# NinV/Background-Debiased-Video-CIL

Measured on AMD Instinct MI355X. Metric: clips/sec fwd+bwd TSM-R50 8x224^2 bs32/GPU, higher is better.
Workload: dtype f32; 1 GPU; TSM-ResNet50 fwd+bwd+SGD step, synthetic 32x8x3x224x224 clips per GPU, 101 classes, SimpleLinear+CrossEntropyLoss, dropout 0.5, random-init weights; fp32 tensors, accumulators and results; conv products: fp32 via 3xbf16 split, 6 MFMA products, fp32 accumulate (dropped terms <= 2^-24 relative); conv_arith=bf16x3, clips_per_gpu=32, global_batch=32, parallelism=dp1

## Files before the change

### background-debiased-video-cil_amd/_lib.py

```python
from __future__ import annotations

import ctypes
import os
from ctypes import POINTER, Structure, c_char_p, c_float, c_int, c_int32, c_int64, c_size_t, c_uint16, c_uint64, c_void_p

_HERE = os.path.dirname(os.path.abspath(__file__))
_OVERRIDE = os.environ.get('BDVCIL_LIB_PATH')
LIB_PATH = _OVERRIDE or os.path.join(_HERE, 'csrc', 'libbdvcil_hip.so')
ABI_VERSION = 32

_lib = None


class ConvGeom(Structure):
    _fields_ = [(n, c_int32) for n in
                ('N', 'H', 'W', 'Cin', 'Ho', 'Wo', 'Cout', 'R', 'S', 'stride', 'pad', 'T', 'fold', 'pad_w', 'Rt', 'st_t', 'act_dtype')]

    def key(self):
        return tuple(getattr(self, n) for n, _ in self._fields_)


P = c_void_p
_F3 = c_float * 3

# ... 2 lines not shown
    _fields_ = [('scale', c_void_p), ('shift', c_void_p), ('residual', c_void_p), ('relu', c_int32)]


class BnStatFuse(Structure):
    _fields_ = [('y', c_void_p), ('relu_mask', c_void_p), ('mean', c_void_p), ('invstd', c_void_p), ('partial', c_void_p),
                ('relu_scale', c_void_p), ('relu_shift', c_void_p)]

class JpegInfo(Structure):
    _fields_ = [('width', c_int32), ('height', c_int32), ('ncomp', c_int32), ('h', c_int32 * 3), ('v', c_int32 * 3),
                ('blocks_w', c_int32 * 3), ('blocks_h', c_int32 * 3), ('down_w', c_int32 * 3), ('down_h', c_int32 * 3),
                ('qt', (c_uint16 * 64) * 3), ('coef_offset', c_int64 * 3), ('coef_count', c_int64)]

    def geometry_key(self):
        return (self.width, self.height, self.ncomp, tuple(self.h), tuple(self.v))


SIGNATURES = {
    'bdv_last_error': (c_char_p, []),
    'bdv_abi_version': (c_int, []),
    'bdv_source_hash': (c_char_p, []),
    'bdv_conv_workspace_bytes': (c_size_t, [POINTER(ConvGeom), c_int]),
    'bdv_conv_fprop_stat_rows': (c_int, [POINTER(ConvGeom)]),
    'bdv_conv_fprop': (c_int, [P, P, P, POINTER(ConvGeom), P, POINTER(ConvAffine), P, c_size_t, P]),
    'bdv_conv_fprop_x3': (c_int, [P, P, P, POINTER(ConvGeom), P, POINTER(ConvAffine), P, c_size_t, P]),
    'bdv_conv_dgrad_stat_rows': (c_int, [POINTER(ConvGeom)]),
    'bdv_conv_dgrad': (c_int, [P, P, P, P, P, POINTER(ConvGeom), POINTER(BnStatFuse), P, c_size_t, P]),
    'bdv_conv_dgrad_x3': (c_int, [P, P, P, P, P, P, POINTER(ConvGeom), POINTER(BnStatFuse), P, c_size_t, P]),
    'bdv_conv_weight_planes_bytes': (c_size_t, [POINTER(ConvGeom)]),
    'bdv_conv_split_weights': (c_int, [P, POINTER(ConvGeom), P, P, P]),
    'bdv_conv_fprop_pre_ok': (c_int, [POINTER(ConvGeom)]),
    'bdv_conv_fprop_pre_stat_rows': (c_int, [POINTER(ConvGeom)]),
    'bdv_conv_wgrad_pre_ok': (c_int, [POINTER(ConvGeom)]),
    'bdv_conv_debug_force_tile': (c_int, [c_int]),
    'bdv_conv_uses_planes': (c_int, [POINTER(ConvGeom), c_int, c_int]),
    'bdv_conv_kernel_name': (c_int, [POINTER(ConvGeom), c_int, c_int, c_char_p, c_size_t]),
    'bdv_conv_fprop_pl_stat_rows': (c_int, [POINTER(ConvGeom), c_int]),
    'bdv_conv_dgrad_pl_stat_rows': (c_int, [POINTER(ConvGeom), c_int]),
    'bdv_conv_fprop_pl': (c_int, [P, P, P, P, POINTER(ConvGeom), P, POINTER(ConvAffine), P, c_size_t, c_int, P, P, P]),
    'bdv_conv_dgrad_pl': (c_int, [P, P, P, P, P, P, POINTER(ConvGeom), POINTER(BnStatFuse), P, c_size_t, c_int, P]),
    'bdv_conv_wgrad': (c_int, [P, P, P, c_float, POINTER(ConvGeom), P, c_size_t, P]),
    'bdv_conv_wgrad_splits': (c_int, [POINTER(ConvGeom)]),
    'bdv_conv_wgrad_partial': (c_int, [P, P, POINTER(ConvGeom), P, c_size_t, P]),
    'bdv_conv_wgrad_partial_x3': (c_int, [P, P, POINTER(ConvGeom), P, c_size_t, P]),
    'bdv_conv_wgrad_pl_splits': (c_int, [POINTER(ConvGeom)]),
    'bdv_conv_wgrad_partial_pl': (c_int, [P, P, POINTER(ConvGeom), P, c_size_t, c_int, P, P, P]),
    'bdv_wgrad_reduce_batched': (c_int, [P, P, P, P, c_int, c_float, P]),
    'bdv_bn_workspace_bytes': (c_size_t, [c_int64, c_int]),
    'bdv_bn_train_stats': (c_int, [P, c_int64, c_int, P, P, c_float, c_float, P, P, P, P, P, P, P, c_size_t, P]),
    'bdv_bn_train_finalize': (c_int, [P, c_int, c_int64, c_int, P, P, c_float, c_float, P, P, P, P, P, P, P]),
    'bdv_bn_eval_params': (c_int, [c_int, P, P, P, P, c_float, P, P, P]),
    'bdv_bn_apply': (c_int, [P, P, P, P, P, P, P, P, c_int64, c_int, c_int, c_int, P]),
    'bdv_bn_backward': (c_int, [P, P, P, P, P, P, P, P, P, c_float, c_int64, c_int, c_int, P, c_int, P, P, P, c_size_t, c_int, P]),
    'bdv_bn_finalize_scratch_bytes': (c_size_t, [c_int]),
    'bdv_bn_finalize_splits': (c_int, [c_int, c_int]),
    'bdv_bn_train_finalize_split': (c_int, [P, c_int, c_int64, c_int, P, P, c_float, c_float, P, P, P, P, P, P, c_int, P, c_size_t, P]),
    'bdv_bn_backward_split': (c_int, [P, P, P, P, P, P, P, P, P, c_float, c_int64, c_int, c_int, P, c_int, P, P, P, c_size_t, c_int,
                                      c_int, P, c_size_t, P]),
    'bdv_bn_pair_workspace_bytes': (c_size_t, [c_int64, c_int]),
    'bdv_bn_backward_pair': (c_int, [P, P, P, P, P, P, P, c_int, P, P, P, P, P, P, P, P, P, P, c_int64, c_int, P, c_size_t, c_int, c_int,
                                     P, c_size_t, P]),
    'bdv_bn_eval_backward': (c_int, [P, P, P, P, P, P, P, P, P, P, P, c_float, c_int64, c_int, P, c_size_t, c_int, c_int, P, c_size_t, P]),
    'bdv_bn_backward_maxpool_split': (c_int, [P, P, P, P, P, P, P, P, P, P, c_float, c_int, c_int, c_int, c_int, P, c_size_t, c_int,
                                              c_int, P, c_size_t, P]),
    'bdv_bn_backward_maxpool': (c_int, [P, P, P, P, P, P, P, P, P, P, c_float, c_int, c_int, c_int, c_int, P, c_size_t, c_int, P]),
    'bdv_relu_bwd': (c_int, [P, P, P, P, c_int64, c_int, P]),
    'bdv_add': (c_int, [P, P, P, c_int64, c_int, P]),
# ... 28 lines not shown
    'bdv_lsc_bwd': (c_int, [P, P, P, P, P, P, P, P, c_float, P, c_int, c_int, c_int, c_int, P]),
    'bdv_linear_fwd': (c_int, [P, P, P, P, c_int, c_int, c_int, P]),
    'bdv_linear_bwd': (c_int, [P, P, P, P, P, P, c_float, c_int, c_int, c_int, P]),
    'bdv_consensus_fwd': (c_int, [P, P, c_int, c_int, c_int, P]),
    'bdv_consensus_bwd': (c_int, [P, P, c_int, c_int, c_int, P]),
    'bdv_dropout': (c_int, [P, P, c_int64, c_float, c_uint64, P]),
    'bdv_lsc_loss': (c_int, [P, P, P, c_float, c_int, P, P, P, P, c_int, c_int, P]),
    'bdv_softce_loss': (c_int, [P, P, P, P, P, c_int, c_int, P]),
    'bdv_icarl_targets': (c_int, [P, P, c_int, P, P, c_int, c_int, P]),
    'bdv_acm_targets': (c_int, [P, P, P, c_float, P, c_int, c_int, P]),
    'bdv_softmax_mean': (c_int, [P, P, c_int, c_int, c_int, c_int, P]),
    'bdv_topk_acc': (c_int, [P, P, P, c_int, c_int, P]),
    'bdv_repr_from_features': (c_int, [P, P, P, c_int, c_int, c_int, c_int, P]),
    'bdv_nme_workspace_bytes': (c_size_t, [c_int, c_int]),
    'bdv_nme_classify': (c_int, [P, P, P, P, c_int, c_int, c_int, c_int, P, c_size_t, P]),
    'bdv_class_means': (c_int, [P, P, P, c_int, c_int, c_int, P]),
    'bdv_herding_workspace_bytes': (c_size_t, [c_int, c_int]),
    'bdv_herding_select': (c_int, [P, c_int, c_int, c_int, c_int, P, P, P, P, c_size_t, P]),
    'bdv_randaug_workspace_bytes': (c_size_t, [c_int, c_int, c_int, c_int]),
    'bdv_randaug_apply': (c_int, [P, P, P, P, c_int, c_int, c_int, c_int, P, c_size_t, P]),
    'bdv_reduce_workspace_bytes': (c_size_t, []),
    'bdv_kd_mse_fwd': (c_int, [P, P, P, c_int64, P, c_size_t, c_int, P]),
    'bdv_kd_mse_bwd': (c_int, [P, P, P, c_float, P, c_int64, c_int, P]),
    'bdv_multi_sqnorm': (c_int, [P, P, c_int, P, P, c_size_t, P]),
    'bdv_clip_coef': (c_int, [P, c_float, c_float, P, P]),
    'bdv_multi_sgd': (c_int, [P, P, P, P, P, P, c_int, c_float, c_float, P, P]),
}


class HipExtensionError(RuntimeError):
    pass


HASHED_SOURCES = ('conv_mfma.hip', 'bn.hip', 'pool_frontend.hip', 'head_loss.hip', 'repr.hip', 'augment.hip', 'optim.hip', 'jpeg.hip',
                  'background.hip', 'actor_cut_mix.hip', 'sim_cam.hip', 'api_common.cpp', 'common.h', 'resize_linear.h', 'Makefile', '../../include/bdvcil_hip.h')


def source_hash():
    import hashlib
    h = hashlib.sha256()
    base = os.path.join(_HERE, 'csrc')
    for name in HASHED_SOURCES:
        path = os.path.join(base, name)
        if not os.path.exists(path):
            return None
        with open(path, 'rb') as f:
            h.update(f.read())
    return h.hexdigest()


def lib():
    global _lib
    if _lib is None:
        if not os.path.exists(LIB_PATH):
            raise HipExtensionError(
                f'HIP extension not built: {LIB_PATH} is missing. Run `python -c "import __graft_entry__ as g; '
                f'g.build()"` (or `make -C {os.path.dirname(LIB_PATH)}`). There is no CPU fallback.')
        handle = ctypes.CDLL(LIB_PATH)
        for name, (res, args) in SIGNATURES.items():
            fn = getattr(handle, name)
            fn.restype = res
            fn.argtypes = args
        if handle.bdv_abi_version() != ABI_VERSION:
            raise HipExtensionError(f'ABI mismatch: library {handle.bdv_abi_version()} != binding {ABI_VERSION}')
        want, have = source_hash(), handle.bdv_source_hash().decode()
        if want is not None and want != have and not _OVERRIDE:
            raise HipExtensionError(f'stale library: {LIB_PATH} was built from other sources (hash {have[:12]}, in-tree '
                                    f'{want[:12]}). Rebuild: make -C {os.path.dirname(LIB_PATH)}')
# ... 9 lines not shown
```

### background-debiased-video-cil_amd/csrc/conv_mfma.hip

```cpp
#include <stdlib.h>
#include "common.h"

#ifdef BDV_STAMPS
__device__ unsigned long long* g_stamp_buf = nullptr;
__device__ int g_stamp_cap = 0;
#define BDV_STAMP(slot)                                                                                                          \
  do {                                                                                                                           \
    if (threadIdx.x == 0 && g_stamp_buf != nullptr && (int)(blockIdx.x + gridDim.x * blockIdx.y) < g_stamp_cap) {                 \
      unsigned long long* q_ = g_stamp_buf + (size_t)(blockIdx.x + gridDim.x * blockIdx.y) * 8;                                  \
      if ((slot) == 4) asm volatile("s_waitcnt vmcnt(0)" ::: "memory");                                                          \
      q_[slot] = __builtin_amdgcn_s_memtime();                                                                                   \
      if ((slot) == 0) { q_[5] = __builtin_amdgcn_s_memrealtime(); q_[7] = __builtin_amdgcn_s_getreg((4 << 0) | (0 << 6) | (31 << 11)); } \
      if ((slot) == 4) q_[6] = __builtin_amdgcn_s_memrealtime();                                                                 \
    }                                                                                                                            \
  } while (0)
#else
#define BDV_STAMP(slot) do { } while (0)
#endif

namespace {

constexpr int BK = 32;

struct Geom {
  int N, H, W, Cin, Ho, Wo, Cout, R, S, stride, pad, pad_w, T, fold;
  int Rt, st_t;
  float rcp_RS, rcp_S;
  int M;
  int Ktot;
  float rcp_HoWo, rcp_Wo;
  int stagger;
};

typedef unsigned int u32x4 __attribute__((ext_vector_type(4)));
// ... 558 lines not shown
      ra[p] = buf_load16(xr, (a_base[p] + koff_a + cls * frame_bytes) | (v ? 0 : kOOB), 0);
    }
#pragma unroll
    for (int p = 0; p < BP; ++p) rb[p] = buf_load16(wr, b_base[p], koff_b);
    s += 1;
    const int ws_ = (s == g.S) ? 1 : 0;
    s = ws_ ? 0 : s;
    r += ws_;
    const int wr_ = (r == g.R) ? 1 : 0;
    r = wr_ ? 0 : r;
    chunk += wr_;
  };

  f32x16 acc[TM][TN];
  zero_acc<TM, TN>(acc);

  load();
  for (int kt = it.kb; kt < it.ke; ++kt) {
    __syncthreads();
    store_transposed<LDA, AP>(As, ra, tid);
    store_transposed<LDB, BP>(Bs, rb, tid);
    __syncthreads();
    if (kt + 1 < it.ke) load();
    mma_stage<LDA, LDB, TM, TN, 32 * WM, 32 * WN, true, true>(As, Bs, acc, wm0, wn0, lane);
  }

  if (it.pslot >= 0) {
    store_partial<TM, TN>(slab, it.pslot, acc, tid);
    return;
  }
  fprop_epilogue<BM, BN, WM, WN>(acc, smem, y, g, epi, mt, nt, tid);
}

typedef __bf16 bf16x8_t __attribute__((ext_vector_type(8)));
typedef __bf16 bf16x4_t __attribute__((ext_vector_type(4)));
typedef float f32x4_t __attribute__((ext_vector_type(4)));
constexpr int X3_LDK = BK + 8;

typedef __bf16 bf16x2_t __attribute__((ext_vector_type(2)));
typedef float f32x2_t __attribute__((ext_vector_type(2)));
typedef unsigned u32x2_t __attribute__((ext_vector_type(2)));
__device__ __forceinline__ unsigned pack_bf16x2(float a, float b) {
  return __builtin_bit_cast(unsigned, __builtin_convertvector((f32x2_t){a, b}, bf16x2_t));
}
__device__ __forceinline__ u32x2_t bf16_hi_pairs(const float4 v) { return (u32x2_t){pack_bf16x2(v.x, v.y), pack_bf16x2(v.z, v.w)}; }
__device__ __forceinline__ void split3_pairs(const float4 v, u32x2_t& hi, u32x2_t& mid, u32x2_t& lo) {
  const unsigned h0 = pack_bf16x2(v.x, v.y), h1 = pack_bf16x2(v.z, v.w);
  const float rx = v.x - __uint_as_float(h0 << 16), ry = v.y - __uint_as_float(h0 & 0xffff0000u);
  const float rz = v.z - __uint_as_float(h1 << 16), rw = v.w - __uint_as_float(h1 & 0xffff0000u);
  const unsigned m0 = pack_bf16x2(rx, ry), m1 = pack_bf16x2(rz, rw);
  const float sx = rx - __uint_as_float(m0 << 16), sy = ry - __uint_as_float(m0 & 0xffff0000u);
  const float sz = rz - __uint_as_float(m1 << 16), sw = rw - __uint_as_float(m1 & 0xffff0000u);
  hi = (u32x2_t){h0, h1};
  mid = (u32x2_t){m0, m1};
  lo = (u32x2_t){pack_bf16x2(sx, sy), pack_bf16x2(sz, sw)};
}

template <int ROWS, int P>
__device__ __forceinline__ void store_split3(unsigned short* __restrict__ dst, const float4 (&v)[P], int tid) {
  const int arow = tid >> 3, kg = tid & 7;
#pragma unroll
  for (int p = 0; p < P; ++p) {
    u32x2_t hi, mid, lo;
    split3_pairs(v[p], hi, mid, lo);
    unsigned short* q = dst + (arow + 32 * p) * X3_LDK + 4 * kg;
    *reinterpret_cast<u32x2_t*>(q) = hi;
    *reinterpret_cast<u32x2_t*>(q + ROWS * X3_LDK) = mid;
    *reinterpret_cast<u32x2_t*>(q + 2 * ROWS * X3_LDK) = lo;
  }
}

template <int TM, int TN, int MS, int NS, int ROWS_A, int ROWS_B>
__device__ __forceinline__ void mma_stage_x3(const unsigned short* __restrict__ As, const unsigned short* __restrict__ Bs,
                                             f32x16 (&acc)[TM][TN], int wm0, int wn0, int lane) {
  const int r = lane & 31, h = lane >> 5;
#pragma unroll
  for (int s = 0; s < BK / 16; ++s) {
    bf16x8_t a[3][TM], b[3][TN];
#pragma unroll
    for (int p = 0; p < 3; ++p) {
#pragma unroll
      for (int i = 0; i < TM; ++i)
        a[p][i] = *reinterpret_cast<const bf16x8_t*>(As + (p * ROWS_A + wm0 + MS * i + r) * X3_LDK + 16 * s + 8 * h);
#pragma unroll
      for (int j = 0; j < TN; ++j)
        b[p][j] = *reinterpret_cast<const bf16x8_t*>(Bs + (p * ROWS_B + wn0 + NS * j + r) * X3_LDK + 16 * s + 8 * h);
    }
#pragma unroll
    for (int i = 0; i < TM; ++i)
// ... 998 lines not shown
    float4* d = reinterpret_cast<float4*>(dw) + i;
    if (beta != 0.f) {
      const float4 o = *d;
      s.x += beta * o.x;
      s.y += beta * o.y;
      s.z += beta * o.z;
      s.w += beta * o.w;
    }
    *d = s;
  }
}

__global__ __launch_bounds__(256) void wgrad_reduce_kernel(const float* __restrict__ slab, float* __restrict__ dw, float beta,
                                                            int splits, int64_t numel4) {
  wgrad_reduce_block(slab, dw, beta, splits, numel4, blockIdx.x);
}

struct ReduceBatch {
  const float* slab[BDV_MAX_REDUCE_ITEMS];
  float* dw[BDV_MAX_REDUCE_ITEMS];
  int splits[BDV_MAX_REDUCE_ITEMS];
  int numel4[BDV_MAX_REDUCE_ITEMS];
  int first_block[BDV_MAX_REDUCE_ITEMS + 1];
  int n;
};

__global__ __launch_bounds__(256) void wgrad_reduce_batched_kernel(ReduceBatch rb, float beta) {
  int k = 0;
  while (k + 1 < rb.n && (int)blockIdx.x >= rb.first_block[k + 1]) ++k;
  wgrad_reduce_block(rb.slab[k], rb.dw[k], beta, rb.splits[k], rb.numel4[k], blockIdx.x - rb.first_block[k]);
}


__device__ __forceinline__ int pl_off(int row, int c) { return row * 64 + ((c ^ ((row >> 2) & 3)) << 4); }

__device__ __forceinline__ void pl_split_store(unsigned char* __restrict__ base, int plane_bytes, int row, int kg, const float4 v) {
  u32x2_t hi, mid, lo;
  split3_pairs(v, hi, mid, lo);
  unsigned char* q = base + pl_off(row, kg >> 1) + 8 * (kg & 1);
  *reinterpret_cast<u32x2_t*>(q) = hi;
  *reinterpret_cast<u32x2_t*>(q + plane_bytes) = mid;
  *reinterpret_cast<u32x2_t*>(q + 2 * plane_bytes) = lo;
}

__device__ __forceinline__ int pl_frag_off(int row0, int s, int lane) {
  const int r = lane & 31, h = lane >> 5;
  return pl_off(row0 + r, 2 * s + h);
}

template <int BM, int BN, int WM, int WN, int NP = 3>
__device__ __forceinline__ void mma_stage_pl(const unsigned char* __restrict__ As, const unsigned char* __restrict__ Bs,
                                             f32x16 (&acc)[BM / WM / 32][BN / WN / 32], const int (&fa)[2], const int (&fb)[2]) {
  constexpr int TM = BM / WM / 32, TN = BN / WN / 32;
  constexpr int PA = BM * 64, PB = BN * 64;
#pragma unroll
  for (int s = 0; s < BK / 16; ++s) {
    bf16x8_t a[NP][TM], b[NP][TN];
#pragma unroll
    for (int p = 0; p < NP; ++p) {
#pragma unroll
      for (int i = 0; i < TM; ++i) a[p][i] = *reinterpret_cast<const bf16x8_t*>(As + fa[s] + (p * PA + 32 * WM * i * 64));
#pragma unroll
      for (int j = 0; j < TN; ++j) b[p][j] = *reinterpret_cast<const bf16x8_t*>(Bs + fb[s] + (p * PB + 32 * WN * j * 64));
    }
#pragma unroll
    for (int i = 0; i < TM; ++i)
#pragma unroll
// ... 930 lines not shown
    p.wk = plan_work_pl(p.MT * p.NT, nk, k.iter_us, p.seg_bytes, ws_bytes, &p.est_us, pl_cfg_round(cfg));
  } else {
    p.wk.dp_tiles = p.MT * p.NT;
    p.wk.rem_tiles = 0;
    p.wk.split = 1;
    p.est_us = (double)((p.MT * p.NT + 255) / 256) * nk * k.iter_us;
  }
  return p;
}

constexpr bool r1_planes_enabled() { return true; }

bool c4_x3_enabled() {
  static const bool on = getenv("BDVCIL_C4_X3") == nullptr || atoi(getenv("BDVCIL_C4_X3")) != 0;
  return on;
}

int pl_fprop_cfg(const bdv_conv_geom* g, int pieces = 3) {
  if (g->Cin % BK != 0) return -1;
  return pl_pick(false, g->Cout, g->R * g->S * g->Cin / BK, g->R * g->S, g->stride, pieces);
}
int pl_dgrad_cfg(const bdv_conv_geom* g, int pieces = 3) {
  if (g->Cout % BK != 0) return -1;
  return pl_pick(true, g->Cin, g->R * g->S * g->Cout / BK, g->R * g->S, g->stride, pieces, g->fold > 0);
}
bool pl_fprop_ok(const bdv_conv_geom* g, int pieces = 3) { return pl_fprop_cfg(g, pieces) >= 0; }
int pl_fprop_cfg_pre(const bdv_conv_geom* g) {
  if (g->Cin % BK != 0 || g->Cout % 64 != 0) return -1;
  const int cfg = pl_fprop_cfg(g, 3);
  if (cfg >= 0) return cfg;
  return g->Cout % 256 == 0 ? 0 : g->Cout % 128 == 0 ? 1 : 3;
}
bool pl_dgrad_ok(const bdv_conv_geom* g, int pieces = 3) { return pl_dgrad_cfg(g, pieces) >= 0; }


struct WgradPlan {
  bool small;
  bool c4;
  int MTw, NTw, splits, kt_per_split;
};

WgradPlan plan_wgrad(const bdv_conv_geom* g) {
  static const int W = getenv("BDVCIL_WGRAD_W") ? atoi(getenv("BDVCIL_WGRAD_W")) : 768;
  WgradPlan p;
  p.c4 = (g->Cin % BK) != 0;
  p.small = p.c4 || (g->Cout % 128) != 0 || (g->Cin % 128) != 0;
  const int bm = p.small ? 64 : 128, bn = p.small ? 64 : 128;
  const int ktot = g->R * g->S * g->Cin;
  p.MTw = g->Cout / bm;
  p.NTw = p.c4 ? (ktot + bn - 1) / bn : g->R * g->S * (g->Cin / bn);
  const int64_t M = (int64_t)g->N * g->Ho * g->Wo;
  const int nkt = (int)((M + BK - 1) / BK);
  const int tiles = p.MTw * p.NTw;
  int best_s = 1;
  double best_cost = 1e30;
  const double dw_bytes = (double)g->Cout * ktot * 4.0;
  const int Wk = p.small ? 2 * W : W;
  for (int k = 1; k <= 4; ++k) {
    int sp = (int)(((long long)k * Wk) / tiles);
    if (sp < 1) sp = 1;
    if (sp > 1024) sp = 1024;
    while (sp > 1 && (nkt + sp - 1) / sp < 4) --sp;
    const int per = (nkt + sp - 1) / sp;
    const double rounds = (double)(((long long)tiles * sp + Wk - 1) / Wk);
    const double t_iter = 1.7 * 3.0 * (p.small ? 0.25 : 1.0);
    const double cost = rounds * per * t_iter + 4.0 + sp * dw_bytes / 4.0e6;
// ... 260 lines not shown
extern "C" int bdv_conv_dgrad(const float* dy, const float* w, float* dx, const float* add_src,
                              const uint32_t* add_mask_src, const bdv_conv_geom* gg, const bdv_bn_stat_fuse* bn_stat,
                              void* workspace, size_t workspace_bytes, void* stream) {
  return conv_dgrad_impl(dy, w, nullptr, dx, add_src, add_mask_src, gg, bn_stat, workspace, workspace_bytes, stream);
}

extern "C" int bdv_conv_dgrad_x3(const float* dy, const float* w, const float* w_t, float* dx, const float* add_src,
                                 const uint32_t* add_mask_src, const bdv_conv_geom* gg, const bdv_bn_stat_fuse* bn_stat,
                                 void* workspace, size_t workspace_bytes, void* stream) {
  BDV_REQUIRE(w_t != nullptr, "bdv_conv_dgrad_x3: w_t is null");
  return conv_dgrad_impl(dy, w, w_t, dx, add_src, add_mask_src, gg, bn_stat, workspace, workspace_bytes, stream);
}

extern "C" size_t bdv_conv_weight_planes_bytes(const bdv_conv_geom* gg) {
  if (check_geom(gg, "bdv_conv_weight_planes_bytes")) return 0;
  return (size_t)3 * gg->Cout * gg->R * gg->S * gg->Cin * sizeof(unsigned short);
}

#ifdef BDV_STAMPS
extern "C" int bdv_debug_set_stamps(void* buf, int cap_workgroups) {
  unsigned long long* p = (unsigned long long*)buf;
  if (hipMemcpyToSymbol(HIP_SYMBOL(g_stamp_buf), &p, sizeof(p)) != hipSuccess) return -1;
  if (hipMemcpyToSymbol(HIP_SYMBOL(g_stamp_cap), &cap_workgroups, sizeof(int)) != hipSuccess) return -1;
  return 0;
}
#endif

extern "C" int bdv_conv_debug_force_tile(int cfg) {
  BDV_REQUIRE(cfg >= -1 && cfg <= kNumPlCfg, "bdv_conv_debug_force_tile: cfg %d (-1 automatic, 0 = 128x256, 1 = 256x128, 2 = 256x256, 3 = 256x64, 4 = 64x128 (dgrad), 5 = 128x128 (four waves), 6 = none)", cfg);
  g_pl_tile_forced = cfg;
  return BDV_OK;
}

extern "C" int bdv_conv_kernel_name(const bdv_conv_geom* gg, int kind, int arith, char* out, size_t n) {
  if (int e = check_geom(gg, "bdv_conv_kernel_name")) return e;
  BDV_REQUIRE(out && n > 0 && kind >= 0 && kind <= 2, "bdv_conv_kernel_name: bad argument");
  const bool c4 = gg->Cin % BK != 0;
  const int pieces = arith == 2 ? 1 : arith == 3 ? 2 : 3;
  if (kind == 0) {
    const int cfg = arith ? pl_fprop_cfg(gg, pieces) : -1;
    if (cfg >= 0) {
      snprintf(out, n, "conv_fprop_pl_kernel<%d, %d, %d, %d, %d, %d>", kPlCfg[cfg].BM, kPlCfg[cfg].BN, pl_cfg_wm(cfg), pl_cfg_wn(cfg), kPlCfg[cfg].nbuf, pieces);
    } else if (c4) {
      snprintf(out, n, "conv_fprop_c4_%skernel<128, %d, 2, 2>", arith && c4_x3_enabled() ? "x3_" : "", gg->Cout % 128 == 0 ? 128 : 64);
    } else if (gg->Cout % 128 == 0 && arith) {
      snprintf(out, n, "conv_fprop_x3_kernel<128, 128, 2, 2, %s>", r1_planes_enabled() ? "true" : "false");
    } else {
      snprintf(out, n, "conv_fprop_kernel<128, %d, 2, 2>", gg->Cout % 128 == 0 ? 128 : 64);
    }
  } else if (kind == 1) {
    const int cfg = arith ? pl_dgrad_cfg(gg, pieces) : -1;
    if (cfg >= 0) {
      snprintf(out, n, "conv_dgrad_pl_kernel<%d, %d, %d, %d, %d, %d>", kPlCfg[cfg].BM, kPlCfg[cfg].BN, pl_cfg_wm(cfg), pl_cfg_wn(cfg), kPlCfg[cfg].nbuf, pieces);
    } else if (gg->Cin % 128 == 0 && arith) {
      snprintf(out, n, "conv_dgrad_x3_kernel<128, 128, 2, 2, %s>", r1_planes_enabled() ? "true" : "false");
    } else {
      snprintf(out, n, "conv_dgrad_kernel<128, %d, 2, 2>", gg->Cin % 128 == 0 ? 128 : 64);
    }
  } else {
    if (arith && pl_wgrad_ok(gg)) {
      const WgradPlPlan p = plan_wgrad_pl(gg);
      snprintf(out, n, "conv_wgrad_pl_kernel<%d, %d", p.BM, p.BN);
    } else {
      const WgradPlan p = plan_wgrad(gg);
      snprintf(out, n, "conv_wgrad_kernel<%d, %d, 2, 2", p.small ? 64 : 128, p.small ? 64 : 128);
    }
  }
  return BDV_OK;
}

extern "C" int bdv_conv_uses_planes(const bdv_conv_geom* gg, int kind, int pieces) {
  if (check_geom(gg, "bdv_conv_uses_planes")) return 0;
  if (kind == 0) return pl_fprop_ok(gg, pieces) || (pieces >= 2 && r1_planes_enabled() && gg->Cin % BK == 0 && gg->Cout % 128 == 0) ? 1 : 0;
  if (kind == 1) return pl_dgrad_ok(gg, pieces) || (pieces >= 2 && r1_planes_enabled() && gg->Cout % BK == 0 && gg->Cin % 128 == 0) ? 1 : 0;
// ... 52 lines not shown
  BDV_REQUIRE_ACT(gg->act_dtype, "bdv_conv_fprop_pl");
  if (h16)
    BDV_REQUIRE(pieces == 1 && !pre && planes_fprop != nullptr && pl_fprop_ok(gg, 1),
                "bdv_conv_fprop_pl: bf16 activation storage needs pieces = 1, the weight planes, Cin %% 32 == 0 and Cout %% 64 == 0 (Cin=%d Cout=%d)", gg->Cin, gg->Cout);
  if (pre) {
    BDV_REQUIRE(pre_shift != nullptr && planes_fprop != nullptr && pieces == 3 && gg->fold == 0 && pl_fprop_cfg_pre(gg) >= 0,
                "bdv_conv_fprop_pl: a producer BatchNorm in the loader needs the plane kernels (pieces 3, no temporal shift, Cin %% 32 == 0)");
    BDV_REQUIRE(bdv_aligned16(pre_scale) && bdv_aligned16(pre_shift), "bdv_conv_fprop_pl: pre_scale / pre_shift must be 16-byte aligned");
  }
  if (!pre && (planes_fprop == nullptr || !pl_fprop_ok(gg, pieces)))
    return conv_fprop_impl((const float*)x, w, (float*)y, gg, bn_partial, affine, workspace, workspace_bytes, stream, true,
                           gg->Cin % BK == 0 && r1_planes_enabled() ? planes_fprop : nullptr);
  BDV_REQUIRE(x && y, "bdv_conv_fprop_pl: null pointer");
  FpropEpi epi = {bn_partial, 0, nullptr, nullptr, nullptr, 0, pre_scale, pre_shift};
  if (affine != nullptr) {
    BDV_REQUIRE(bn_partial == nullptr, "bdv_conv_fprop_pl: batch statistics and the folded eval-mode BatchNorm exclude each other");
    BDV_REQUIRE(affine->scale && affine->shift, "bdv_conv_fprop_pl: null pointer in bdv_conv_affine");
    BDV_REQUIRE(bdv_aligned16(affine->scale) && bdv_aligned16(affine->shift) && bdv_aligned16(affine->residual),
                "bdv_conv_fprop_pl: bdv_conv_affine pointers must be 16-byte aligned");
    epi.scale = affine->scale;
    epi.shift = affine->shift;
    epi.res = affine->residual;
    epi.relu = affine->relu;
  }
  BDV_REQUIRE(bdv_aligned16(x) && bdv_aligned16(planes_fprop) && bdv_aligned16(y) && bdv_aligned16(workspace),
              "bdv_conv_fprop_pl: pointers must be 16-byte aligned");
  Geom g = make_geom(gg);
  g.M = g.N * g.Ho * g.Wo;
  g.Ktot = g.Rt * g.R * g.S * g.Cin;
  BDV_REQUIRE((int64_t)3 * g.Cout * g.Ktot * 2 < (1ll << 31), "bdv_conv_fprop_pl: weight planes exceed 2^31 bytes");
  hipStream_t s = (hipStream_t)stream;
  const PlPlan p = plan_pl(pre ? pl_fprop_cfg_pre(gg) : pl_fprop_cfg(gg, pieces), g.M, g.Cout, g.Ktot / BK, workspace ? (workspace_bytes < kMaxSplitWorkspace ? workspace_bytes : kMaxSplitWorkspace) : 0, !h16);
  BDV_REQUIRE(p.cfg >= 0, "bdv_conv_fprop_pl: no tile configuration for Cout=%d", g.Cout);
  const int blocks = p.wk.dp_tiles + p.wk.rem_tiles * p.wk.split;
  epi.MT = p.MT;
  float* slab = (float*)workspace;
  const unsigned short* wp = (const unsigned short*)planes_fprop;
  if (debug_plan())
    fprintf(stderr, "[bdv plan] fprop_pl %dx%d Cin %d Cout %d k%d s%d: cfg %d tiles %d nk %d -> dp %d rem %d split %d (est %.0f us)\n", g.H,
            g.W, g.Cin, g.Cout, g.R, g.stride, p.cfg, p.MT * p.NT, p.nk, p.wk.dp_tiles, p.wk.rem_tiles, p.wk.split, p.est_us);
#define BDV_FPROP_PL(BM_, BN_, WM_, WN_, NB_)                                                                                         \
  do {                                                                                                                                \
    if (h16)                                                                                                                          \
      hipLaunchKernelGGL((conv_fprop_pl_kernel<BM_, BN_, WM_, WN_, NB_, 1, false, 2>), dim3(blocks), dim3(64 * WM_ * WN_), 0, s, x, wp, y, \
                         g, p.NT, p.wk, slab, epi);                                                                                   \
    else if (pre)                                                                                                                     \
      hipLaunchKernelGGL((conv_fprop_pl_kernel<BM_, BN_, WM_, WN_, NB_, 3, true>), dim3(blocks), dim3(64 * WM_ * WN_), 0, s, x, wp, y,  \
                         g, p.NT, p.wk, slab, epi);                                                                                   \
    else if (pieces == 1)                                                                                                             \
      hipLaunchKernelGGL((conv_fprop_pl_kernel<BM_, BN_, WM_, WN_, NB_, 1>), dim3(blocks), dim3(64 * WM_ * WN_), 0, s, x, wp, y, g,    \
                         p.NT, p.wk, slab, epi);                                                                                      \
    else if (pieces == 2)                                                                                                             \
      hipLaunchKernelGGL((conv_fprop_pl_kernel<BM_, BN_, WM_, WN_, NB_, 2>), dim3(blocks), dim3(64 * WM_ * WN_), 0, s, x, wp, y, g,    \
                         p.NT, p.wk, slab, epi);                                                                                      \
    else                                                                                                                              \
      hipLaunchKernelGGL((conv_fprop_pl_kernel<BM_, BN_, WM_, WN_, NB_, 3>), dim3(blocks), dim3(64 * WM_ * WN_), 0, s, x, wp, y, g,    \
                         p.NT, p.wk, slab, epi);                                                                                      \
    BDV_LAUNCH_CHECK("bdv_conv_fprop_pl");                                                                                            \
    if (p.wk.split > 1) {                                                                                                             \
      hipLaunchKernelGGL((conv_fprop_fixup_kernel<BM_, BN_, WM_, WN_>), dim3(p.wk.rem_tiles), dim3(64 * WM_ * WN_), 0, s,             \
                         (const float*)slab, (float*)y, g, p.NT, p.wk, epi);                                                                  \
      BDV_LAUNCH_CHECK("bdv_conv_fprop_pl(fixup)");                                                                                   \
    }                                                                                                                                 \
  } while (0)
  if (p.cfg == 0) BDV_FPROP_PL(128, 256, 2, 4, 2);
  else if (p.cfg == 1) BDV_FPROP_PL(256, 128, 4, 2, 2);
// ... 280 lines not shown
```

### include/bdvcil_hip.h

```cpp
#ifndef BDVCIL_HIP_H
#define BDVCIL_HIP_H

#include <stddef.h>
#include <stdint.h>

#ifdef __cplusplus
extern "C" {
#endif

#define BDV_OK 0
#define BDV_EINVAL (-1)
#define BDV_EWORKSPACE (-2)

#define BDV_ACT_F32 0
#define BDV_ACT_BF16 1

typedef struct bdv_conv_geom {
  int32_t N;
  int32_t H, W;
  int32_t Cin;
  int32_t Ho, Wo;
  int32_t Cout;
  int32_t R, S;
  int32_t stride;
// ... 14 lines not shown
int bdv_conv_fprop_stat_rows(const bdv_conv_geom* g);
typedef struct bdv_conv_affine {
  const float* scale;
  const float* shift;
  const void* residual;
  int32_t relu;
} bdv_conv_affine;
int bdv_conv_fprop(const float* x, const float* w, float* y, const bdv_conv_geom* g, float* bn_partial,
                   const bdv_conv_affine* affine, void* workspace, size_t workspace_bytes, void* stream);
int bdv_conv_fprop_x3(const float* x, const float* w, float* y, const bdv_conv_geom* g, float* bn_partial,
                      const bdv_conv_affine* affine, void* workspace, size_t workspace_bytes, void* stream);

typedef struct bdv_bn_stat_fuse {
  const void* y;
  const uint32_t* relu_mask;
  const float* mean;
  const float* invstd;
  float* partial;
  const float* relu_scale;
  const float* relu_shift;
} bdv_bn_stat_fuse;
int bdv_conv_dgrad_stat_rows(const bdv_conv_geom* g);

int bdv_conv_dgrad(const float* dy, const float* w, float* dx, const float* add_src,
                   const uint32_t* add_mask_src, const bdv_conv_geom* g, const bdv_bn_stat_fuse* bn_stat, void* workspace,
                   size_t workspace_bytes, void* stream);
int bdv_conv_dgrad_x3(const float* dy, const float* w, const float* w_t, float* dx, const float* add_src,
                      const uint32_t* add_mask_src, const bdv_conv_geom* g, const bdv_bn_stat_fuse* bn_stat, void* workspace,
                      size_t workspace_bytes, void* stream);

size_t bdv_conv_weight_planes_bytes(const bdv_conv_geom* g);
int bdv_conv_split_weights(const float* w, const bdv_conv_geom* g, void* planes_fprop, void* planes_dgrad, void* stream);
int bdv_conv_debug_force_tile(int cfg);
int bdv_conv_uses_planes(const bdv_conv_geom* g, int kind, int pieces);
int bdv_conv_kernel_name(const bdv_conv_geom* g, int kind, int arith, char* out, size_t n);
int bdv_conv_fprop_pl_stat_rows(const bdv_conv_geom* g, int pieces);
int bdv_conv_dgrad_pl_stat_rows(const bdv_conv_geom* g, int pieces);
int bdv_conv_fprop_pl(const void* x, const float* w, const void* planes_fprop, void* y, const bdv_conv_geom* g,
                      float* bn_partial, const bdv_conv_affine* affine, void* workspace, size_t workspace_bytes, int pieces,
                      const float* pre_scale, const float* pre_shift, void* stream);
int bdv_conv_fprop_pre_ok(const bdv_conv_geom* g);
int bdv_conv_fprop_pre_stat_rows(const bdv_conv_geom* g);
int bdv_conv_dgrad_pl(const void* dy, const float* w, const void* planes_dgrad, void* dx, const void* add_src,
                      const uint32_t* add_mask_src, const bdv_conv_geom* g, const bdv_bn_stat_fuse* bn_stat, void* workspace,
                      size_t workspace_bytes, int pieces, void* stream);

int bdv_conv_wgrad(const float* dy, const float* x, float* dw, float beta, const bdv_conv_geom* g, void* workspace,
                   size_t workspace_bytes, void* stream);
#define BDV_MAX_REDUCE_ITEMS 32
int bdv_conv_wgrad_splits(const bdv_conv_geom* g);
int bdv_conv_wgrad_partial(const float* dy, const float* x, const bdv_conv_geom* g, void* slab, size_t slab_bytes,
                           void* stream);
int bdv_wgrad_reduce_batched(const float* const* slabs, float* const* dws, const int* splits, const int64_t* numels, int n,
                             float beta, void* stream);
int bdv_conv_wgrad_pl_splits(const bdv_conv_geom* g);
int bdv_conv_wgrad_partial_pl(const void* dy, const void* x, const bdv_conv_geom* g, void* slab, size_t slab_bytes,
                              int pieces, const float* pre_scale, const float* pre_shift, void* stream);
int bdv_conv_wgrad_pre_ok(const bdv_conv_geom* g);
int bdv_conv_wgrad_partial_x3(const float* dy, const float* x, const bdv_conv_geom* g, void* slab, size_t slab_bytes,
                              void* stream);

size_t bdv_bn_workspace_bytes(int64_t M, int C);
int bdv_bn_train_stats(const float* y, int64_t M, int C, const float* gamma, const float* beta,
                       float eps, float momentum, float* running_mean, float* running_var,
                       float* save_mean, float* save_invstd, float* scale, float* shift,
                       void* workspace, size_t workspace_bytes, void* stream);
// ... 159 lines not shown
```

Measured before the change: 620.3 clips/s.

## Add persistent streaming kernel for 64->256 1x1 conv fprop with register-resident weights

```diff
diff --git a/background-debiased-video-cil_amd/_lib.py b/background-debiased-video-cil_amd/_lib.py
--- a/background-debiased-video-cil_amd/_lib.py
+++ b/background-debiased-video-cil_amd/_lib.py
@@ -58,6 +58,7 @@
     'bdv_conv_fprop_pre_stat_rows': (c_int, [POINTER(ConvGeom)]),
     'bdv_conv_wgrad_pre_ok': (c_int, [POINTER(ConvGeom)]),
     'bdv_conv_debug_force_tile': (c_int, [c_int]),
+    'bdv_conv_debug_stream1x1': (c_int, [c_int, c_int]),
     'bdv_conv_uses_planes': (c_int, [POINTER(ConvGeom), c_int, c_int]),
     'bdv_conv_kernel_name': (c_int, [POINTER(ConvGeom), c_int, c_int, c_char_p, c_size_t]),
     'bdv_conv_fprop_pl_stat_rows': (c_int, [POINTER(ConvGeom), c_int]),
@@ -152,8 +153,8 @@
     pass
 
 
-HASHED_SOURCES = ('conv_mfma.hip', 'bn.hip', 'pool_frontend.hip', 'head_loss.hip', 'repr.hip', 'augment.hip', 'optim.hip', 'jpeg.hip',
-                  'background.hip', 'actor_cut_mix.hip', 'sim_cam.hip', 'api_common.cpp', 'common.h', 'resize_linear.h', 'Makefile', '../../include/bdvcil_hip.h')
+HASHED_SOURCES = ('conv_mfma.hip', 'conv_stream1x1.hip', 'bn.hip', 'pool_frontend.hip', 'head_loss.hip', 'repr.hip', 'augment.hip', 'optim.hip', 'jpeg.hip',
+                  'background.hip', 'actor_cut_mix.hip', 'sim_cam.hip', 'api_common.cpp', 'common.h', 'conv_pieces.h', 'conv_stream1x1.h', 'resize_linear.h', 'Makefile', '../../include/bdvcil_hip.h')
 
 
 def source_hash():
diff --git a/background-debiased-video-cil_amd/csrc/conv_mfma.hip b/background-debiased-video-cil_amd/csrc/conv_mfma.hip
--- a/background-debiased-video-cil_amd/csrc/conv_mfma.hip
+++ b/background-debiased-video-cil_amd/csrc/conv_mfma.hip
@@ -1,5 +1,7 @@
 #include <stdlib.h>
 #include "common.h"
+#include "conv_pieces.h"
+#include "conv_stream1x1.h"
 
 #ifdef BDV_STAMPS
 __device__ unsigned long long* g_stamp_buf = nullptr;
@@ -624,29 +626,10 @@
   fprop_epilogue<BM, BN, WM, WN>(acc, smem, y, g, epi, mt, nt, tid);
 }
 
-typedef __bf16 bf16x8_t __attribute__((ext_vector_type(8)));
 typedef __bf16 bf16x4_t __attribute__((ext_vector_type(4)));
 typedef float f32x4_t __attribute__((ext_vector_type(4)));
 constexpr int X3_LDK = BK + 8;
 
-typedef __bf16 bf16x2_t __attribute__((ext_vector_type(2)));
-typedef float f32x2_t __attribute__((ext_vector_type(2)));
-typedef unsigned u32x2_t __attribute__((ext_vector_type(2)));
-__device__ __forceinline__ unsigned pack_bf16x2(float a, float b) {
-  return __builtin_bit_cast(unsigned, __builtin_convertvector((f32x2_t){a, b}, bf16x2_t));
-}
-__device__ __forceinline__ u32x2_t bf16_hi_pairs(const float4 v) { return (u32x2_t){pack_bf16x2(v.x, v.y), pack_bf16x2(v.z, v.w)}; }
-__device__ __forceinline__ void split3_pairs(const float4 v, u32x2_t& hi, u32x2_t& mid, u32x2_t& lo) {
-  const unsigned h0 = pack_bf16x2(v.x, v.y), h1 = pack_bf16x2(v.z, v.w);
-  const float rx = v.x - __uint_as_float(h0 << 16), ry = v.y - __uint_as_float(h0 & 0xffff0000u);
-  const float rz = v.z - __uint_as_float(h1 << 16), rw = v.w - __uint_as_float(h1 & 0xffff0000u);
-  const unsigned m0 = pack_bf16x2(rx, ry), m1 = pack_bf16x2(rz, rw);
-  const float sx = rx - __uint_as_float(m0 << 16), sy = ry - __uint_as_float(m0 & 0xffff0000u);
-  const float sz = rz - __uint_as_float(m1 << 16), sw = rw - __uint_as_float(m1 & 0xffff0000u);
-  hi = (u32x2_t){h0, h1};
-  mid = (u32x2_t){m0, m1};
-  lo = (u32x2_t){pack_bf16x2(sx, sy), pack_bf16x2(sz, sw)};
-}
 
 template <int ROWS, int P>
 __device__ __forceinline__ void store_split3(unsigned short* __restrict__ dst, const float4 (&v)[P], int tid) {
@@ -1711,7 +1694,6 @@
 }
 
 
-__device__ __forceinline__ int pl_off(int row, int c) { return row * 64 + ((c ^ ((row >> 2) & 3)) << 4); }
 
 __device__ __forceinline__ void pl_split_store(unsigned char* __restrict__ base, int plane_bytes, int row, int kg, const float4 v) {
   u32x2_t hi, mid, lo;
@@ -2708,6 +2690,13 @@
   return g->Cout % 256 == 0 ? 0 : g->Cout % 128 == 0 ? 1 : 3;
 }
 bool pl_dgrad_ok(const bdv_conv_geom* g, int pieces = 3) { return pl_dgrad_cfg(g, pieces) >= 0; }
+
+bool stream1x1_fprop_route(const bdv_conv_geom* g, int pieces) {
+  const int pad_w = g->pad_w < 0 ? g->pad : g->pad_w;
+  return pieces == 3 && bdv_stream1x1::enabled() && pl_tile_override() < 0 && g->act_dtype == BDV_ACT_F32 && g->R == 1 && g->S == 1 &&
+         g->stride == 1 && g->pad == 0 && pad_w == 0 && g->fold == 0 && g->Rt <= 1 && g->Cin == bdv_stream1x1::kCin &&
+         g->Cout == bdv_stream1x1::kCout;
+}
 
 
 struct WgradPlan {
@@ -3034,6 +3023,12 @@
   return BDV_OK;
 }
 
+extern "C" int bdv_conv_debug_stream1x1(int enable, int max_workgroups) {
+  BDV_REQUIRE((enable == 0 || enable == 1) && max_workgroups >= 0, "bdv_conv_debug_stream1x1: enable %d (0 | 1), max_workgroups %d (0 = one per CU)", enable, max_workgroups);
+  bdv_stream1x1::configure(enable, max_workgroups);
+  return BDV_OK;
+}
+
 extern "C" int bdv_conv_kernel_name(const bdv_conv_geom* gg, int kind, int arith, char* out, size_t n) {
   if (int e = check_geom(gg, "bdv_conv_kernel_name")) return e;
   BDV_REQUIRE(out && n > 0 && kind >= 0 && kind <= 2, "bdv_conv_kernel_name: bad argument");
@@ -3041,7 +3036,9 @@
   const int pieces = arith == 2 ? 1 : arith == 3 ? 2 : 3;
   if (kind == 0) {
     const int cfg = arith ? pl_fprop_cfg(gg, pieces) : -1;
-    if (cfg >= 0) {
+    if (arith && stream1x1_fprop_route(gg, pieces)) {
+      snprintf(out, n, "conv_stream1x1_fprop_kernel");
+    } else if (cfg >= 0) {
       snprintf(out, n, "conv_fprop_pl_kernel<%d, %d, %d, %d, %d, %d>", kPlCfg[cfg].BM, kPlCfg[cfg].BN, pl_cfg_wm(cfg), pl_cfg_wn(cfg), kPlCfg[cfg].nbuf, pieces);
     } else if (c4) {
       snprintf(out, n, "conv_fprop_c4_%skernel<128, %d, 2, 2>", arith && c4_x3_enabled() ? "x3_" : "", gg->Cout % 128 == 0 ? 128 : 64);
@@ -3160,6 +3157,10 @@
   hipStream_t s = (hipStream_t)stream;
   const PlPlan p = plan_pl(pre ? pl_fprop_cfg_pre(gg) : pl_fprop_cfg(gg, pieces), g.M, g.Cout, g.Ktot / BK, workspace ? (workspace_bytes < kMaxSplitWorkspace ? workspace_bytes : kMaxSplitWorkspace) : 0, !h16);
   BDV_REQUIRE(p.cfg >= 0, "bdv_conv_fprop_pl: no tile configuration for Cout=%d", g.Cout);
+  if (!pre && affine == nullptr && stream1x1_fprop_route(gg, pieces)) {
+    if (debug_plan()) fprintf(stderr, "[bdv plan] fprop_pl %dx%d Cin %d Cout %d k1 s1: stream1x1, %d row tiles\n", g.H, g.W, g.Cin, g.Cout, p.MT);
+    return bdv_stream1x1::fprop_launch((const float*)x, (const unsigned short*)planes_fprop, (float*)y, g.M, bn_partial, s);
+  }
   const int blocks = p.wk.dp_tiles + p.wk.rem_tiles * p.wk.split;
   epi.MT = p.MT;
   float* slab = (float*)workspace;
diff --git a/background-debiased-video-cil_amd/csrc/conv_pieces.h b/background-debiased-video-cil_amd/csrc/conv_pieces.h
--- /dev/null
+++ b/background-debiased-video-cil_amd/csrc/conv_pieces.h
@@ -0,0 +1,25 @@
+#pragma once
+#include <hip/hip_runtime.h>
+
+typedef __bf16 bf16x8_t __attribute__((ext_vector_type(8)));
+typedef __bf16 bf16x2_t __attribute__((ext_vector_type(2)));
+typedef float f32x2_t __attribute__((ext_vector_type(2)));
+typedef unsigned u32x2_t __attribute__((ext_vector_type(2)));
+
+__device__ __forceinline__ unsigned pack_bf16x2(float a, float b) {
+  return __builtin_bit_cast(unsigned, __builtin_convertvector((f32x2_t){a, b}, bf16x2_t));
+}
+__device__ __forceinline__ u32x2_t bf16_hi_pairs(const float4 v) { return (u32x2_t){pack_bf16x2(v.x, v.y), pack_bf16x2(v.z, v.w)}; }
+__device__ __forceinline__ void split3_pairs(const float4 v, u32x2_t& hi, u32x2_t& mid, u32x2_t& lo) {
+  const unsigned h0 = pack_bf16x2(v.x, v.y), h1 = pack_bf16x2(v.z, v.w);
+  const float rx = v.x - __uint_as_float(h0 << 16), ry = v.y - __uint_as_float(h0 & 0xffff0000u);
+  const float rz = v.z - __uint_as_float(h1 << 16), rw = v.w - __uint_as_float(h1 & 0xffff0000u);
+  const unsigned m0 = pack_bf16x2(rx, ry), m1 = pack_bf16x2(rz, rw);
+  const float sx = rx - __uint_as_float(m0 << 16), sy = ry - __uint_as_float(m0 & 0xffff0000u);
+  const float sz = rz - __uint_as_float(m1 << 16), sw = rw - __uint_as_float(m1 & 0xffff0000u);
+  hi = (u32x2_t){h0, h1};
+  mid = (u32x2_t){m0, m1};
+  lo = (u32x2_t){pack_bf16x2(sx, sy), pack_bf16x2(sz, sw)};
+}
+
+__device__ __forceinline__ int pl_off(int row, int c) { return row * 64 + ((c ^ ((row >> 2) & 3)) << 4); }
diff --git a/background-debiased-video-cil_amd/csrc/conv_stream1x1.h b/background-debiased-video-cil_amd/csrc/conv_stream1x1.h
--- /dev/null
+++ b/background-debiased-video-cil_amd/csrc/conv_stream1x1.h
@@ -0,0 +1,14 @@
+#pragma once
+#include <hip/hip_runtime.h>
+#include <stdint.h>
+
+namespace bdv_stream1x1 {
+
+constexpr int kCin = 64, kCout = 256, kRows = 128;
+
+bool enabled();
+void configure(int enable, int max_workgroups);
+
+int fprop_launch(const float* x, const unsigned short* planes, float* y, int M, float* bn_partial, hipStream_t stream);
+
+}
diff --git a/background-debiased-video-cil_amd/csrc/conv_stream1x1.hip b/background-debiased-video-cil_amd/csrc/conv_stream1x1.hip
--- /dev/null
+++ b/background-debiased-video-cil_amd/csrc/conv_stream1x1.hip
@@ -0,0 +1,185 @@
+#include "common.h"
+#include "conv_pieces.h"
+#include "conv_stream1x1.h"
+
+namespace {
+
+typedef unsigned int u32x4 __attribute__((ext_vector_type(4)));
+
+constexpr int kThreads = 512;
+constexpr int kPlane = bdv_stream1x1::kRows * 64;
+constexpr int kStep = 3 * kPlane;
+constexpr int kStage = 2 * kStep;
+constexpr int kTileInBytes = bdv_stream1x1::kRows * bdv_stream1x1::kCin * 4;
+constexpr int kRowOutBytes = bdv_stream1x1::kCout * 4;
+constexpr int kWeightPlane = bdv_stream1x1::kCout * bdv_stream1x1::kCin * 2;
+
+__global__ __launch_bounds__(kThreads, 1) void conv_stream1x1_fprop_kernel(const float* __restrict__ x,
+                                                                          const unsigned short* __restrict__ wp,
+                                                                          float* __restrict__ y, int M, int ntiles,
+                                                                          float* __restrict__ bn_partial) {
+  __shared__ __attribute__((aligned(16))) unsigned char smem[2 * kStage];
+  const int tid = threadIdx.x;
+  const int lane = tid & 63, wave = tid >> 6;
+  const int c = lane & 31, h = lane >> 5;
+  const int col = 32 * wave + c;
+  const bool late = wave >= 4;
+
+  const __amdgpu_buffer_rsrc_t xr = __builtin_amdgcn_make_buffer_rsrc((void*)x, 0, M * (bdv_stream1x1::kCin * 4), 0x00020000);
+  const __amdgpu_buffer_rsrc_t yr = __builtin_amdgcn_make_buffer_rsrc((void*)y, 0, M * kRowOutBytes, 0x00020000);
+  const __amdgpu_buffer_rsrc_t wr = __builtin_amdgcn_make_buffer_rsrc((void*)wp, 0, 3 * kWeightPlane, 0x00020000);
+
+  bf16x8_t wf[2][2][3];
+#pragma unroll
+  for (int ks = 0; ks < 2; ++ks)
+#pragma unroll
+    for (int s = 0; s < 2; ++s)
+#pragma unroll
+      for (int p = 0; p < 3; ++p)
+        wf[ks][s][p] = __builtin_bit_cast(
+            bf16x8_t, __builtin_amdgcn_raw_buffer_load_b128(wr, (ks * bdv_stream1x1::kCout + col) * 64 + (2 * s + h) * 16 + p * kWeightPlane, 0, 0));
+
+  const int ld_off = tid * 16;
+  const int arow = tid >> 4, unit = tid & 15;
+  const int st_off = (unit >> 3) * kStep + pl_off(arow, (unit & 7) >> 1) + 8 * (unit & 1);
+  const int fa[2] = {pl_off(c, h), pl_off(c, 2 + h)};
+
+  float4 ra[4];
+  auto load = [&](int tile) __attribute__((always_inline)) {
+    const int base = tile * kTileInBytes + ld_off;
+#pragma unroll
+    for (int p = 0; p < 4; ++p) {
+      const u32x4 v = __builtin_amdgcn_raw_buffer_load_b128(xr, base + 8192 * p, 0, 0);
+      ra[p] = make_float4(__uint_as_float(v.x), __uint_as_float(v.y), __uint_as_float(v.z), __uint_as_float(v.w));
+    }
+  };
+  auto split_store = [&](int stage) __attribute__((always_inline)) {
+    unsigned char* const q = smem + stage * kStage + st_off;
+#pragma unroll
+    for (int p = 0; p < 4; ++p) {
+      u32x2_t hi, mid, lo;
+      split3_pairs(ra[p], hi, mid, lo);
+      *reinterpret_cast<u32x2_t*>(q + 2048 * p) = hi;
+      *reinterpret_cast<u32x2_t*>(q + 2048 * p + kPlane) = mid;
+      *reinterpret_cast<u32x2_t*>(q + 2048 * p + 2 * kPlane) = lo;
+    }
+  };
+  auto compute = [&](int stage, int tile) __attribute__((always_inline)) {
+    const unsigned char* const As = smem + stage * kStage;
+    f32x16 acc[4];
+#pragma unroll
+    for (int i = 0; i < 4; ++i)
+#pragma unroll
+      for (int e = 0; e < 16; ++e) acc[i][e] = 0.f;
+#pragma unroll
+    for (int ks = 0; ks < 2; ++ks)
+#pragma unroll
+      for (int s = 0; s < 2; ++s) {
+        bf16x8_t a[3][4];
+#pragma unroll
+        for (int p = 0; p < 3; ++p)
+#pragma unroll
+          for (int i = 0; i < 4; ++i) a[p][i] = *reinterpret_cast<const bf16x8_t*>(As + fa[s] + (ks * kStep + p * kPlane + i * 2048));
+#pragma unroll
+        for (int i = 0; i < 4; ++i) {
+          acc[i] = __builtin_amdgcn_mfma_f32_32x32x16_bf16(a[1][i], wf[ks][s][1], acc[i], 0, 0, 0);
+          acc[i] = __builtin_amdgcn_mfma_f32_32x32x16_bf16(a[0][i], wf[ks][s][2], acc[i], 0, 0, 0);
+          acc[i] = __builtin_amdgcn_mfma_f32_32x32x16_bf16(a[2][i], wf[ks][s][0], acc[i], 0, 0, 0);
+          acc[i] = __builtin_amdgcn_mfma_f32_32x32x16_bf16(a[0][i], wf[ks][s][1], acc[i], 0, 0, 0);
+          acc[i] = __builtin_amdgcn_mfma_f32_32x32x16_bf16(a[1][i], wf[ks][s][0], acc[i], 0, 0, 0);
+          acc[i] = __builtin_amdgcn_mfma_f32_32x32x16_bf16(a[0][i], wf[ks][s][0], acc[i], 0, 0, 0);
+        }
+      }
+    const int ybase = tile * (bdv_stream1x1::kRows * kRowOutBytes) + 4 * h * kRowOutBytes + col * 4;
+#pragma unroll
+    for (int i = 0; i < 4; ++i)
+#pragma unroll
+      for (int e = 0; e < 16; ++e)
+        __builtin_amdgcn_raw_buffer_store_b32(__float_as_uint(acc[i][e]), yr, ybase + (32 * i + (e & 3) + 8 * (e >> 2)) * kRowOutBytes, 0, 0);
+    if (bn_partial != nullptr) {
+      float cs[2], cq[2];
+#pragma unroll
+      for (int wm = 0; wm < 2; ++wm) {
+        cs[wm] = 0.f + acc[wm][0];
+        cs[wm] += acc[wm][1];
+        cq[wm] = __builtin_fmaf(acc[wm][0], acc[wm][0], __fmul_rn(acc[wm][1], acc[wm][1]));
+#pragma unroll
+        for (int i = wm; i < 4; i += 2)
+#pragma unroll
+          for (int e = (i == wm ? 2 : 0); e < 16; ++e) {
+            const float v = acc[i][e];
+            cs[wm] += v;
+            cq[wm] = __builtin_fmaf(v, v, cq[wm]);
+          }
+        cs[wm] += __shfl_xor(cs[wm], 32, 64);
+        cq[wm] += __shfl_xor(cq[wm], 32, 64);
+      }
+      if (h == 0) {
+        float sa = 0.f, sb = 0.f;
+        sa += cs[0];
+        sb += cq[0];
+        sa += cs[1];
+        sb += cq[1];
+        bn_partial[(size_t)tile * bdv_stream1x1::kCout + col] = sa;
+        bn_partial[((size_t)ntiles + tile) * bdv_stream1x1::kCout + col] = sb;
+      }
+    }
+  };
+
+  const int G = gridDim.x;
+  int t = blockIdx.x;
+  load(t);
+  split_store(0);
+  load(t + G);
+  __syncthreads();
+  for (int stage = 0; t < ntiles; t += G, stage ^= 1) {
+    if (late) {
+      split_store(stage ^ 1);
+      load(t + 2 * G);
+      compute(stage, t);
+    } else {
+      compute(stage, t);
+      split_store(stage ^ 1);
+      load(t + 2 * G);
+    }
+    __syncthreads();
+  }
+}
+
+
+int g_enabled = 1;
+int g_max_workgroups = 0;
+
+int cu_count() {
+  static const int n = [] {
+    int dev = 0, v = 0;
+    if (hipGetDevice(&dev) != hipSuccess || hipDeviceGetAttribute(&v, hipDeviceAttributeMultiprocessorCount, dev) != hipSuccess || v <= 0) {
+      (void)hipGetLastError();
+      return 256;
+    }
+    return v;
+  }();
+  return n;
+}
+
+}
+
+namespace bdv_stream1x1 {
+
+bool enabled() { return g_enabled != 0; }
+
+void configure(int enable, int max_workgroups) {
+  g_enabled = enable;
+  g_max_workgroups = max_workgroups;
+}
+
+int fprop_launch(const float* x, const unsigned short* planes, float* y, int M, float* bn_partial, hipStream_t stream) {
+  const int ntiles = (M + kRows - 1) / kRows;
+  int grid = ntiles < cu_count() ? ntiles : cu_count();
+  if (g_max_workgroups > 0 && grid > g_max_workgroups) grid = g_max_workgroups;
+  hipLaunchKernelGGL(conv_stream1x1_fprop_kernel, dim3(grid), dim3(kThreads), 0, stream, x, planes, y, M, ntiles, bn_partial);
+  BDV_LAUNCH_CHECK("bdv_conv_fprop_pl(stream1x1)");
+  return BDV_OK;
+}
+
+}
diff --git a/include/bdvcil_hip.h b/include/bdvcil_hip.h
--- a/include/bdvcil_hip.h
+++ b/include/bdvcil_hip.h
@@ -70,6 +70,7 @@
 size_t bdv_conv_weight_planes_bytes(const bdv_conv_geom* g);
 int bdv_conv_split_weights(const float* w, const bdv_conv_geom* g, void* planes_fprop, void* planes_dgrad, void* stream);
 int bdv_conv_debug_force_tile(int cfg);
+int bdv_conv_debug_stream1x1(int enable, int max_workgroups);
 int bdv_conv_uses_planes(const bdv_conv_geom* g, int kind, int pieces);
 int bdv_conv_kernel_name(const bdv_conv_geom* g, int kind, int arith, char* out, size_t n);
 int bdv_conv_fprop_pl_stat_rows(const bdv_conv_geom* g, int pieces);
```

Measured after the change: 624.4 clips/s, median of 6. About the same (+0.7%).
